# ImChouOWO/A-lightweight-Unsupervised-Feature-Extractor-

Hardware: NVIDIA B200
Metric: tracked frames/sec at N=64 boxes; ROIAlign achieved HBM GB/s vs B200 peak (higher is better)
Workload: dtype f32

## Files before the change

### a-lightweight-unsupervised-feature-extractor-_b200/csrc/tracker.cu

```cuda
#include <stdlib.h>
#include <string.h>

#include <new>

#include <cuda_fp16.h>

#include "assoc_cost.cuh"
#include "kalman.cuh"
#include "lsap.cuh"

namespace b200 {
namespace trk {

struct Span {
    int k;
    __device__ explicit Span(int kk) : k(kk) { B200_SPAN_BEGIN(k); }
    __device__ ~Span() { B200_SPAN_END(k); }
};

#ifdef B200_TRK_TIMING
__device__ long long g_timing[32];
#define TRK_STAMP(k) do { __syncthreads(); if (threadIdx.x == 0 && blockIdx.x == 0) g_timing[k] = clock64(); } while (0)
#define TRK_GSTAMP(k) do { __syncthreads(); if (threadIdx.x == 0 && blockIdx.x == 0 && blockIdx.y == 0) g_timing[16 + (k)] = (long long)::b200::gtime(); } while (0)
#else
// ... 68 lines not shown
    }
    return base;
}

__device__ __forceinline__ void load_kf(const Dev& d, size_t slot, double* x, double* P) {
    const double2* px = reinterpret_cast<const double2*>(d.kf_x + slot * 8);
    const double2* pP = reinterpret_cast<const double2*>(d.kf_P + slot * 64);
#pragma unroll
    for (int k = 0; k < 4; ++k) { const double2 v = px[k]; x[2 * k] = v.x; x[2 * k + 1] = v.y; }
#pragma unroll
    for (int k = 0; k < 32; ++k) { const double2 v = pP[k]; P[2 * k] = v.x; P[2 * k + 1] = v.y; }
}
__device__ __forceinline__ void store_kf(const Dev& d, size_t slot, const double* x, const double* P) {
    double2* px = reinterpret_cast<double2*>(d.kf_x + slot * 8);
    double2* pP = reinterpret_cast<double2*>(d.kf_P + slot * 64);
#pragma unroll
    for (int k = 0; k < 4; ++k) px[k] = make_double2(x[2 * k], x[2 * k + 1]);
#pragma unroll
    for (int k = 0; k < 32; ++k) pP[k] = make_double2(P[2 * k], P[2 * k + 1]);
}

__device__ inline void purge(const Dev& d, int s, int nl, int* scratch) {
    int* order = d.order + (size_t)s * d.MT;
    int* tmp = d.tmp + (size_t)s * d.MT;
    int* fl = d.free_list + (size_t)s * d.MT;
    int* hdr = d.hdr + s * kHdr;
    const size_t sb = (size_t)s * d.MT;
    for (int i = threadIdx.x; i < nl; i += blockDim.x) tmp[i] = order[i];
    __syncthreads();
    const int nfree = hdr[H_NFREE];
    const int keep = block_compact(nl, [&](int i) { return d.miss[sb + tmp[i]] <= d.max_age; },
                                   [&](int pos, int i) { order[pos] = tmp[i]; }, scratch);
    const int dead = block_compact(nl, [&](int i) { return d.miss[sb + tmp[i]] > d.max_age; },
                                   [&](int pos, int i) { fl[nfree + pos] = tmp[i]; }, scratch);
    if (threadIdx.x == 0) { hdr[H_NLIVE] = keep; hdr[H_NFREE] = nfree + dead; }
    __syncthreads();
}

__device__ inline void enqueue_cost_work(int2* work, int* counter, int s, int M, int N, int* scratch) {
    const int tiles = (N + cost::kTileN - 1) / cost::kTileN, total = M * tiles;
    if (total <= 0) return;
    __syncthreads();
    if (threadIdx.x == 0) scratch[0] = atomicAdd(counter, total);
    __syncthreads();
    const int base = scratch[0];
    for (int i = threadIdx.x; i < total; i += blockDim.x) work[base + i] = make_int2(s, (i / tiles) * 64 + i % tiles);
}

__device__ inline void prep_detections(const Dev& d, int s, int n, int part = 0, int nparts = 1) {
    const size_t db = (size_t)s * d.MD;
    const int tid = threadIdx.x;
    const int nw = blockDim.x >> 5, nt = blockDim.x;
    for (int j = part * nw + (tid >> 5); j < n; j += nparts * nw) {
        const float4 v = reinterpret_cast<const float4*>(d.embs + (db + j) * cost::kD)[tid & 31];
        reinterpret_cast<float4*>(d.det_unit + (db + j) * cost::kD)[tid & 31] = cost::unit_row(v);
    }
    for (int j = part * nt + tid; j < n; j += nparts * nt) {
        double b[4];
        float z[4];
#pragma unroll
        for (int k = 0; k < 4; ++k) { b[k] = d.boxes[(db + j) * 4 + k]; d.det_boxf[(db + j) * 4 + k] = (float)b[k]; }
        kf::box_to_z(b, z);
#pragma unroll
        for (int k = 0; k < 4; ++k) d.det_z[(db + j) * 4 + k] = z[k];
        d.det_conff[db + j] = (float)d.confs[db + j];
        d.det_used[db + j] = 0;
    }
}

__device__ inline void predict_slot(const Dev& d, size_t slot) {
    const float q[8] = {1.f, 1.f, 1.f, 1.f, 100.f, 100.f, 100.f, 100.f};
    const float rdiag[4] = {1.f, 1.f, 1.f, 1.f};
    double x[8], P[64], b[4];
    load_kf(d, slot, x, P);
    const int st = d.kf_stage[slot];
    kf::predict(x, P, st, q);
    store_kf(d, slot, x, P);
    kf::x_to_box(x, b);
#pragma unroll
    for (int k = 0; k < 4; ++k) { d.last_bbox[slot * 4 + k] = b[k]; d.prev_boxf[slot * 4 + k] = (float)b[k]; }
    d.prev_conff[slot] = (float)d.last_conf[slot];
    kf::Gate g;
    kf::gate_prepare(x, P, st, rdiag, &g);
#pragma unroll
    for (int k = 0; k < 16; ++k) d.gate_SI[slot * 16 + k] = g.SI[k];
}

__global__ void __launch_bounds__(kThreads) begin_kernel(Dev d) {
    Span span((d.frame_id[0] & 7) * 6 + 0);
    __shared__ int scratch[kThreads / 32];
    const int s = blockIdx.x, tid = threadIdx.x;
    int* hdr = d.hdr + s * kHdr;
    int* cnt = d.cnt + s * kHdr;
    int* res = d.result + (size_t)s * d.res_stride;
    const size_t sb = (size_t)s * d.MT, db = (size_t)s * d.MD;
    const int n = d.n_det[s], nl = hdr[H_NLIVE];
    int* order = d.order + sb;
    if (blockIdx.y == 1) {
        if (n <= 0) return;
        prep_detections(d, s, n);
        return;
    }
    if (s == 0 && tid == 0) d.wcount[2] = 0;
    if (n < 0) {
        if (tid == 0) {
            cnt[C_MODE] = MODE_SKIP;
            res[R_NMATCH] = res[R_NUT] = res[R_NUD] = res[R_STATUS] = res[R_M1] = res[R_M2] = 0;
            res[R_NLIVE] = nl;
            res[R_NEXT] = hdr[H_NEXT];
        }
        return;
    }
    if (n == 0) {
        int* ut = res_ut(d, res);
        for (int p = tid; p < nl; p += blockDim.x) {
            const size_t slot = sb + order[p];
            d.miss[slot] += 1;
            ut[p] = d.tid[slot];
        }
        __syncthreads();
        purge(d, s, nl, scratch);
        if (tid == 0) {
            cnt[C_MODE] = MODE_EMPTY;
            res[R_NMATCH] = 0; res[R_NUT] = nl; res[R_NUD] = 0; res[R_STATUS] = 0; res[R_M1] = res[R_M2] = 0;
            res[R_NLIVE] = hdr[H_NLIVE];
            res[R_NEXT] = hdr[H_NEXT];
        }
        return;
    }
    for (int p = tid; p < nl; p += blockDim.x) predict_slot(d, sb + order[p]);
    int* rm = d.rows_main + sb;
    int* rr = d.rows_reid + sb;
    const int M1 = block_compact(nl, [&](int i) { return d.miss[sb + order[i]] <= d.lost_reid_after; },
                                 [&](int pos, int i) { rm[pos] = order[i]; }, scratch);
    const int M2 = block_compact(nl, [&](int i) { return d.miss[sb + order[i]] > d.lost_reid_after; },
                                 [&](int pos, int i) { rr[pos] = order[i]; }, scratch);
    if (tid == 0) {
        cnt[C_M1] = M1; cnt[C_M2] = M2; cnt[C_NU] = 0; cnt[C_MODE] = MODE_NORMAL;
        cnt[C_NMATCH] = 0; cnt[C_NUT] = 0; cnt[C_STATUS] = 0;
    }
    enqueue_cost_work(d.work1, d.wcount + 0, s, M1, 1, scratch);
}

__device__ inline void cost2_item(const Dev& d, int s, int r, int j0, float* smem, int* s_idx) {
    const int tid = threadIdx.x, warp = tid >> 5, lane = tid & 31;
    const int N = d.cnt[s * kHdr + C_NU];
    const size_t sb = (size_t)s * d.MT, db = (size_t)s * d.MD;
    const size_t slot = sb + d.rows_reid[sb + r];
    int T = d.bank_len[slot];
    const float* rows = d.bank + slot * d.HIST * cost::kD;
    if (T <= 0) { rows = d.ema + slot * cost::kD; T = 1; }
    if (tid < cost::kTileN) {
        const int j = j0 + tid;
        s_idx[tid] = j < N ? d.ud1[db + j] : 0;
    }
    __syncthreads();
    const int tc = cost::bank_cap(T);
    float* sBank = smem;
    float* sDet = sBank + tc * cost::kD;
    float* sSim = sDet + cost::kTileN * cost::kDetStride;
    for (int t = warp; t < tc; t += cost::kThreads / 32) {
        float4 v = make_float4(0, 0, 0, 0);
        if (t < T) v = cost::unit_row(reinterpret_cast<const float4*>(rows + (size_t)t * cost::kD)[lane]);
        reinterpret_cast<float4*>(sBank + t * cost::kD)[lane] = v;
    }
    for (int j = warp; j < cost::kTileN; j += cost::kThreads / 32) {
// ... 82 lines not shown
        float pb[4];
#pragma unroll
        for (int k = 0; k < 4; ++k) pb[k] = d.prev_boxf[slot * 4 + k];
        const float pconf = d.prev_conff[slot];
        float inv0 = 0.0f, inv1 = 0.0f;
        bool have_norm = false;
        RowMin rmin;
        for (int j0 = 0; j0 < N; j0 += 32) {
            const int j = j0 + lane;
            bool alive = false;
            if (j < N) alive = !(kf::gate_d2(SI, xs, stage, d.det_z + (db + j) * 4) > d.maha_thr);
            unsigned todo = __ballot_sync(0xffffffffu, alive);
            float c_app = 0.0f;
            while (todo) {
                const int jl = __ffs(todo) - 1;
                todo &= todo - 1;
                const float4 dv = reinterpret_cast<const float4*>(d.det_unit + (db + j0 + jl) * cost::kD)[lane];
                float s0 = kNegInf, s1 = kNegInf;
                for (int t0 = 0; t0 < T; t0 += 8) {
                    float4 bv[8];
#pragma unroll
                    for (int u = 0; u < 8; ++u)
                        if (t0 + u < T) bv[u] = reinterpret_cast<const float4*>(rows + (size_t)(t0 + u) * cost::kD)[lane];
#pragma unroll
                    for (int u = 0; u < 8; ++u) {
                        const int t = t0 + u;
                        if (t >= T) break;
                        float p = bv[u].x * dv.x;
                        p = fmaf(bv[u].y, dv.y, p); p = fmaf(bv[u].z, dv.z, p); p = fmaf(bv[u].w, dv.w, p);
                        p = warp_sum(p);
                        if (!have_norm) {
                            float q = bv[u].x * bv[u].x;
                            q = fmaf(bv[u].y, bv[u].y, q); q = fmaf(bv[u].z, bv[u].z, q); q = fmaf(bv[u].w, bv[u].w, q);
                            q = warp_sum(q);
                            const float iv = __fdiv_rn(1.0f, __fadd_rn(sqrtf(q), 1e-12f));
                            if (lane == (t & 31)) { if (t < 32) inv0 = iv; else inv1 = iv; }
                        }
                        if (lane == (t & 31)) { if (t < 32) s0 = p; else s1 = p; }
                    }
                }
                have_norm = true;
                if (lane < T) s0 *= inv0;
                if (lane + 32 < T) s1 *= inv1;
                float sum = 0.0f;
                for (int q = 0; q < kk; ++q) {
                    const float mine = fmaxf(s0, s1);
                    const unsigned m = __reduce_max_sync(0xffffffffu, fkey(mine));
                    const unsigned who = __ballot_sync(0xffffffffu, fkey(mine) == m);
                    if (lane == __ffs(who) - 1) {
                        if (s0 >= s1) s0 = kNegInf; else s1 = kNegInf;
                    }
                    const unsigned bits = m ^ ((m >> 31) ? 0x80000000u : 0xffffffffu);
                    sum = __fadd_rn(sum, __uint_as_float(bits));
                }
                const float ca = __fsub_rn(1.0f, __fdiv_rn(sum, (float)kk));
                if (lane == jl) c_app = ca;
            }
            if (j < N) {
                float total_c = 1e9f;
                if (alive)
                    total_c = cost::pair_cost(pb, d.det_boxf + (db + j) * 4, pconf, d.det_conff[db + j], d.pw, c_app).total;
                d.C1[(sb + r) * d.MD + j] = total_c;
                d.C1T[(db + j) * d.MT + r] = total_c;
                rmin.see(total_c, j);
            }
        }
        rmin.finish(d.row_fc + sb + r, d.row_fv + sb + r, lane);
    }
}

__device__ __forceinline__ void transpose_reduce32(float (&p)[32]) {
    const int lane = threadIdx.x & 31;
#pragma unroll
    for (int o = 16; o > 0; o >>= 1) {
        const bool up = lane & o;
#pragma unroll
        for (int i = 0; i < o; ++i) {
            const float keep = up ? p[i + o] : p[i], send = up ? p[i] : p[i + o];
            p[i] = keep + __shfl_xor_sync(0xffffffffu, send, o);
        }
    }
}

template <bool FLY>
__device__ __forceinline__ void cost1_row32(const Dev& d, int s, int r, size_t slot, int N, int lane) {
    const float kNegInf = -__int_as_float(0x7f800000);
    const size_t sb = (size_t)s * d.MT, db = (size_t)s * d.MD;
    int T = d.bank_len[slot];
    const float* rows = d.bank + slot * d.HIST * cost::kD;
    if (T <= 0) { rows = d.ema + slot * cost::kD; T = 1; }
    const int kk = min(d.topk, T);
    double SI[16], xs[4];
#pragma unroll
    for (int k = 0; k < 16; ++k) SI[k] = d.gate_SI[slot * 16 + k];
#pragma unroll
    for (int k = 0; k < 4; ++k) xs[k] = d.kf_x[slot * 8 + k];
    const int stage = d.kf_stage[slot];
    float pb[4];
#pragma unroll
    for (int k = 0; k < 4; ++k) pb[k] = d.prev_boxf[slot * 4 + k];
    const float pconf = d.prev_conff[slot];
    float4 bv[32];
    float inv = 0.0f;
    bool have_bank = false;
    RowMin rmin;
    for (int j0 = 0; j0 < N; j0 += 32) {
        const int j = j0 + lane;
        bool alive = false;
        float zl[4], bf[4];
        float cf = 0.0f;
        if (j < N) {
            if (FLY) {
                double b[4];
#pragma unroll
                for (int k = 0; k < 4; ++k) { b[k] = d.boxes[(db + j) * 4 + k]; bf[k] = (float)b[k]; }
                kf::box_to_z(b, zl);
                cf = (float)d.confs[db + j];
                alive = !(kf::gate_d2(SI, xs, stage, zl) > d.maha_thr);
            } else {
                alive = !(kf::gate_d2(SI, xs, stage, d.det_z + (db + j) * 4) > d.maha_thr);
            }
        }
        unsigned todo = __ballot_sync(0xffffffffu, alive);
        float c_app = 0.0f;
        float4 dv_first = make_float4(0, 0, 0, 0);
        if (todo) {
            const int jf = __ffs(todo) - 1;
            if (FLY) dv_first = reinterpret_cast<const float4*>(d.embs + (db + j0 + jf) * cost::kD)[lane];
            else dv_first = reinterpret_cast<const float4*>(d.det_unit + (db + j0 + jf) * cost::kD)[lane];
        }
        if (todo && !have_bank) {
            float q[32];
#pragma unroll
            for (int t = 0; t < 32; ++t)
                bv[t] = t < T ? reinterpret_cast<const float4*>(rows + (size_t)t * cost::kD)[lane] : make_float4(0, 0, 0, 0);
#pragma unroll
            for (int t = 0; t < 32; ++t) {
                float a = bv[t].x * bv[t].x;
                a = fmaf(bv[t].y, bv[t].y, a); a = fmaf(bv[t].z, bv[t].z, a); a = fmaf(bv[t].w, bv[t].w, a);
                q[t] = a;
            }
            transpose_reduce32(q);
            inv = __fdiv_rn(1.0f, __fadd_rn(sqrtf(q[0]), 1e-12f));
            have_bank = true;
        }
        bool first = true;
        while (todo) {
            const int jl = __ffs(todo) - 1;
            todo &= todo - 1;
            float4 dv = dv_first;
            if (!first) {
                if (FLY) dv = reinterpret_cast<const float4*>(d.embs + (db + j0 + jl) * cost::kD)[lane];
                else dv = reinterpret_cast<const float4*>(d.det_unit + (db + j0 + jl) * cost::kD)[lane];
            }
            first = false;
            if (FLY) dv = cost::unit_row(dv);
            float p[32];
#pragma unroll
            for (int t = 0; t < 32; ++t) {
                float a = bv[t].x * dv.x;
                a = fmaf(bv[t].y, dv.y, a); a = fmaf(bv[t].z, dv.z, a); a = fmaf(bv[t].w, dv.w, a);
                p[t] = a;
            }
            transpose_reduce32(p);
            float sim = lane < T ? p[0] * inv : kNegInf;
            float sum = 0.0f;
            for (int q = 0; q < kk; ++q) {
                const unsigned m = __reduce_max_sync(0xffffffffu, fkey(sim));
                const unsigned who = __ballot_sync(0xffffffffu, fkey(sim) == m);
                if (lane == __ffs(who) - 1) sim = kNegInf;
                const unsigned bits = m ^ ((m >> 31) ? 0x80000000u : 0xffffffffu);
                sum = __fadd_rn(sum, __uint_as_float(bits));
            }
            const float ca = __fsub_rn(1.0f, __fdiv_rn(sum, (float)kk));
            if (lane == jl) c_app = ca;
        }
        if (j < N) {
            float total_c = 1e9f;
            if (alive) {
                if (FLY) total_c = cost::pair_cost(pb, bf, pconf, cf, d.pw, c_app).total;
                else total_c = cost::pair_cost(pb, d.det_boxf + (db + j) * 4, pconf, d.det_conff[db + j], d.pw, c_app).total;
            }
            d.C1[(sb + r) * d.MD + j] = total_c;
            d.C1T[(db + j) * d.MT + r] = total_c;
            rmin.see(total_c, j);
        }
    }
    rmin.finish(d.row_fc + sb + r, d.row_fv + sb + r, lane);
}

__global__ void __launch_bounds__(kCost1Warps * 32, 2) cost1_sparse32_kernel(Dev d) {
    Span span((d.frame_id[0] & 7) * 6 + 1);
    TRK_PDL_PROLOGUE();
    const int total = d.wcount[0];
    const int warp = threadIdx.x >> 5, lane = threadIdx.x & 31;
    for (int wi = blockIdx.x * kCost1Warps + warp; wi < total; wi += gridDim.x * kCost1Warps) {
        const int2 item = d.work1[wi];
        const int s = item.x, r = item.y >> 6;
        const size_t sb = (size_t)s * d.MT;
        cost1_row32<false>(d, s, r, sb + d.rows_main[sb + r], d.n_det[s], lane);
    }
}

__device__ inline void note_matches(const Dev& d, int s, int nm, const int* rows, const float* C, int ldc,
                                    const int* m_col, int reid_stage, int* scratch, int queue_base = -1) {
    if (nm <= 0) return;
    const size_t sb = (size_t)s * d.MT, db = (size_t)s * d.MD;
    const int frame = d.frame_id[s];
    int base = queue_base;
    if (queue_base < 0) {
        __syncthreads();
        if (threadIdx.x == 0) scratch[0] = atomicAdd(d.wcount + 2, nm);
        __syncthreads();
        base = scratch[0];
    }
    for (int qd = threadIdx.x; qd < nm; qd += blockDim.x) {
        const int r = d.m_row[sb + qd], j = d.m_det[sb + qd];
        const size_t slot = sb + rows[r];
        const float c = C[(size_t)r * ldc + m_col[qd]];
#pragma unroll
        for (int k = 0; k < 4; ++k) d.last_bbox[slot * 4 + k] = d.boxes[(db + j) * 4 + k];
        d.last_conf[slot] = d.confs[db + j];
        d.last_frame[slot] = frame;
        d.age[slot] += 1;
        d.miss[slot] = 0;
        d.last_cost[slot] = (double)c;
        d.upd_slot[base + qd] = (int)slot;
        d.upd_det[base + qd] = (int)(db + j);
        d.upd_cost[base + qd] = c;
        d.upd_flag[base + qd] = (uint8_t)reid_stage;
    }
}

constexpr int kUpdWarps = 4;

__device__ __forceinline__ void update_entries(const Dev& d, int first, int total, int wq, int nwq, double* scratch) {
    const int lane = threadIdx.x & 31, sub = lane & 7, grp = lane >> 3;
    double* sP = scratch + (size_t)grp * 96;
    double* sK = sP + 64;
    const float rdiag[4] = {1.f, 1.f, 1.f, 1.f};
    for (int w0 = wq * 4; w0 < total; w0 += nwq * 4) {
        const int idx = first + w0 + grp;
        const bool on = w0 + grp < total;
        size_t slot = 0, det = 0;
        int st = -1, reid = 0;
        double c = 0.0, conf = 0.0;
        if (on) {
            slot = (size_t)d.upd_slot[idx];
            det = (size_t)d.upd_det[idx];
            c = (double)d.upd_cost[idx];
            reid = d.upd_flag[idx];
            st = d.kf_stage[slot];
            conf = d.confs[det];
        }
        const float* z = d.det_z + det * 4;
        const double cmax = reid ? d.reid_only_cost_max : d.cost_update_max;
        int app = on && !(conf < d.conf_update_min) && !(c > cmax);
        const int nst = st < 2 ? st + 1 : 2;
        float4 e[4], o[4];
        size_t slots[4];
        int len[4], head[4];
#pragma unroll
        for (int u = 0; u < 4; ++u) {
            const bool on_u = __shfl_sync(0xffffffffu, (int)on, u * 8) != 0;
            const unsigned long long sl = __shfl_sync(0xffffffffu, (unsigned long long)slot, u * 8);
            const unsigned long long dt = __shfl_sync(0xffffffffu, (unsigned long long)det, u * 8);
            slots[u] = (size_t)sl;
            if (on_u) {
                e[u] = reinterpret_cast<const float4*>(d.det_unit + (size_t)dt * cost::kD)[lane];
                o[u] = reinterpret_cast<const float4*>(d.ema + slots[u] * cost::kD)[lane];
// ... 155 lines not shown
            n_match = block_compact(M, is_match, [&](int pos, int r) {
                const int jl = col[r], j = STAGE == 1 ? jl : d.ud1[db + jl];
                d.m_row[sb + pos] = r;
                d.m_det[sb + pos] = j;
                m_col[pos] = jl;
                d.det_used[db + j] = 1;
                out_m[2 * (match0 + pos)] = d.tid[sb + rows[r]];
                out_m[2 * (match0 + pos) + 1] = j;
            }, scratch);
            n_ut = block_compact(M, [&](int r) { return !is_match(r); }, [&](int pos, int r) {
                const size_t slot = sb + rows[r];
                d.miss[slot] += 1;
                out_ut[ut0 + pos] = d.tid[slot];
            }, scratch);
            __syncthreads();
            note_matches(d, s, n_match, rows, C, d.MD, m_col, STAGE == 2, scratch, OWNQ ? (int)sb + match0 : -1);
        }
    } else if (M > 0) {
        for (int r = tid; r < M; r += blockDim.x) {
            const size_t slot = sb + rows[r];
            d.miss[slot] += 1;
            out_ut[ut0 + r] = d.tid[slot];
        }
        n_ut = M;
        __syncthreads();
    }

    if (STAGE == 1) {
        if (failed) {
            if (tid == 0) { cnt[C_NU] = 0; cnt[C_NMATCH] = 0; cnt[C_NUT] = 0; }
            return true;
        }
        n_left = block_compact(N, [&](int j) { return d.det_used[db + j] == 0; },
                               [&](int pos, int j) { d.ud1[db + pos] = j; }, scratch);
        if (tid == 0) { cnt[C_NU] = n_left; cnt[C_NMATCH] = n_match; cnt[C_NUT] = n_ut; }
        if (!INLINE) enqueue_cost_work(d.work2, d.wcount + 1, s, n_left > 0 ? cnt[C_M2] : 0, n_left, scratch);
        TRK_STAMP(5);
        __syncthreads();
        return false;
    }

    if (failed) {
        if (tid == 0) {
            res[R_NMATCH] = match0; res[R_NUT] = ut0; res[R_NUD] = 0;
            res[R_NLIVE] = hdr[H_NLIVE]; res[R_NEXT] = hdr[H_NEXT]; res[R_STATUS] = cnt[C_STATUS];
            res[R_M1] = cnt[C_M1]; res[R_M2] = cnt[C_M2];
        }
        return true;
    }
    int* out_ud = res_ud(d, res);
    n_left = block_compact(N, [&](int jl) { return d.det_used[db + d.ud1[db + jl]] == 0; },
                           [&](int pos, int jl) { out_ud[pos] = d.ud1[db + jl]; }, scratch);
    int* born = d.born + db;
    const int want = block_compact(n_left, [&](int k) { return !(d.confs[db + out_ud[k]] < d.init_conf_min); },
                                   [&](int pos, int k) { born[pos] = out_ud[k]; }, scratch);
    const int nl = hdr[H_NLIVE];
    const int nb = spawn_tracks(d, s, born, want);
    purge(d, s, nl + nb, scratch);
    if (tid == 0) {
        res[R_NMATCH] = match0 + n_match;
        res[R_NUT] = ut0 + n_ut;
        res[R_NUD] = n_left;
        res[R_NLIVE] = hdr[H_NLIVE];
        res[R_NEXT] = hdr[H_NEXT];
        res[R_STATUS] = cnt[C_STATUS];
        res[R_M1] = cnt[C_M1];
        res[R_M2] = cnt[C_M2];
    }
    return true;
}

template <int STAGE>
__global__ void __launch_bounds__(kThreads) assign_kernel(Dev d, int smem_matrix_floats) {
    Span span((d.frame_id[0] & 7) * 6 + (STAGE == 1 ? 2 : 4));
    TRK_PDL_PROLOGUE();
    extern __shared__ __align__(16) unsigned char smem_raw[];
    assign_body<STAGE, false, false>(d, blockIdx.x, smem_raw, smem_matrix_floats);
}

#ifndef B200_TRK_FRONT_WARPS
#define B200_TRK_FRONT_WARPS 4
#endif
constexpr int kFrontWarps = B200_TRK_FRONT_WARPS;

__global__ void __launch_bounds__(kFrontWarps * 32, 2) front_kernel(Dev d) {
    Span span((d.frame_id[0] & 7) * 6 + 0);
    extern __shared__ __align__(16) int s_rows[];
    __shared__ int scratch[kThreads / 32];
    const int s = blockIdx.y, g = blockIdx.x, G = gridDim.x, tid = threadIdx.x, warp = tid >> 5, lane = tid & 31;
    TRK_GSTAMP(0);
    int* hdr = d.hdr + s * kHdr;
    int* cnt = d.cnt + s * kHdr;
    int* res = d.result + (size_t)s * d.res_stride;
    const size_t sb = (size_t)s * d.MT;
    const int n = d.n_det[s], nl = hdr[H_NLIVE];
    const int* order = d.order + sb;
    if (s == 0 && g == 0 && tid == 0) d.wcount[2] = 0;
    if (n < 0) {
        if (g == 0 && tid == 0) {
            cnt[C_MODE] = MODE_SKIP;
            res[R_NMATCH] = res[R_NUT] = res[R_NUD] = res[R_STATUS] = res[R_M1] = res[R_M2] = 0;
            res[R_NLIVE] = nl;
            res[R_NEXT] = hdr[H_NEXT];
        }
        return;
    }
    if (n == 0) {
        if (g != 0) return;
        int* ut = res_ut(d, res);
        for (int p = tid; p < nl; p += blockDim.x) {
            const size_t slot = sb + order[p];
            d.miss[slot] += 1;
            ut[p] = d.tid[slot];
        }
        __syncthreads();
        purge(d, s, nl, scratch);
        if (tid == 0) {
            cnt[C_MODE] = MODE_EMPTY;
            res[R_NMATCH] = 0; res[R_NUT] = nl; res[R_NUD] = 0; res[R_STATUS] = 0; res[R_M1] = res[R_M2] = 0;
            res[R_NLIVE] = hdr[H_NLIVE];
            res[R_NEXT] = hdr[H_NEXT];
        }
        return;
    }
    int* rm = s_rows;
    int* rr = s_rows + d.MT;
    const int M1 = block_compact(nl, [&](int i) { return d.miss[sb + order[i]] <= d.lost_reid_after; },
                                 [&](int pos, int i) { rm[pos] = order[i]; }, scratch);
    const int M2 = block_compact(nl, [&](int i) { return d.miss[sb + order[i]] > d.lost_reid_after; },
                                 [&](int pos, int i) { rr[pos] = order[i]; }, scratch);
    if (g == 0) {
        for (int i = tid; i < M1; i += blockDim.x) d.rows_main[sb + i] = rm[i];
        for (int i = tid; i < M2; i += blockDim.x) d.rows_reid[sb + i] = rr[i];
        if (tid == 0) {
            cnt[C_M1] = M1; cnt[C_M2] = M2; cnt[C_NU] = 0; cnt[C_MODE] = MODE_NORMAL;
            cnt[C_NMATCH] = 0; cnt[C_NUT] = 0; cnt[C_STATUS] = 0;
        }
    }
    TRK_GSTAMP(1);
    prep_detections(d, s, n, g, G);
    const int own1 = M1 > g ? (M1 - g + G - 1) / G : 0, own2 = M2 > g ? (M2 - g + G - 1) / G : 0;
    for (int i = tid; i < own1 + own2; i += blockDim.x)
        predict_slot(d, sb + (i < own1 ? rm[g + i * G] : rr[g + (i - own1) * G]));
    __syncthreads();
    TRK_GSTAMP(2);
    for (int i = warp; i < own1; i += kFrontWarps) {
        const int r = g + i * G;
        cost1_row32<true>(d, s, r, sb + rm[r], n, lane);
    }
    TRK_GSTAMP(3);
}

#ifndef B200_TRK_BACK_CLUSTER
#define B200_TRK_BACK_CLUSTER 4
#endif
constexpr int kBackCluster = B200_TRK_BACK_CLUSTER;

__device__ __forceinline__ unsigned cluster_ctarank() {
    unsigned r;
    asm volatile("mov.u32 %0, %%cluster_ctarank;" : "=r"(r));
    return r;
}
__device__ __forceinline__ unsigned cluster_nctarank() {
    unsigned r;
    asm volatile("mov.u32 %0, %%cluster_nctarank;" : "=r"(r));
    return r;
}
__device__ __forceinline__ void cluster_sync_all() {
    asm volatile("barrier.cluster.arrive.release.aligned;\n\tbarrier.cluster.wait.acquire.aligned;" ::: "memory");
}

template <bool UPDATES>
__global__ void __launch_bounds__(kThreads, UPDATES ? 1 : 2) back_kernel(Dev d, int smem_matrix_floats) {
    Span span((d.frame_id[0] & 7) * 6 + 2);
    TRK_PDL_PROLOGUE();
    extern __shared__ __align__(16) unsigned char smem_raw[];
    __shared__ int s_idx[cost::kTileN];
    const unsigned rank = cluster_ctarank(), nrank = cluster_nctarank();
    const int s = blockIdx.x / nrank, tid = threadIdx.x;
    const int* cnt = d.cnt + s * kHdr;
    TRK_GSTAMP(4);
    if (rank == 0) {
        if (!assign_body<1, true, UPDATES>(d, s, smem_raw, smem_matrix_floats)) {
            TRK_GSTAMP(5);
            const int M2 = cnt[C_M2], NU = cnt[C_NU];
            if (M2 > 0 && NU > 0) {
                const int tiles = (NU + cost::kTileN - 1) / cost::kTileN;
                for (int it = 0; it < M2 * tiles; ++it)
                    cost2_item(d, s, it / tiles, (it % tiles) * cost::kTileN, reinterpret_cast<float*>(smem_raw), s_idx);
            }
            __syncthreads();
        }
        TRK_GSTAMP(6);
        assign_body<2, true, UPDATES>(d, s, smem_raw, smem_matrix_floats);
        __syncthreads();
        TRK_GSTAMP(7);
    }
    if (!UPDATES) return;
    if (nrank > 1) cluster_sync_all();
    if (cnt[C_MODE] != MODE_NORMAL) return;
    const int total = d.result[(size_t)s * d.res_stride + R_NMATCH];
    const int warp = tid >> 5;
    update_entries(d, (int)((size_t)s * d.MT), total, (int)rank * (kThreads / 32) + warp, (int)nrank * (kThreads / 32),
                   reinterpret_cast<double*>(smem_raw) + (size_t)warp * 4 * 96);
    TRK_GSTAMP(8);
}


__device__ inline int find_slot(const Dev& d, int s, int nl, int track_id) {
    const size_t sb = (size_t)s * d.MT;
    int lo = 0, hi = nl - 1;
    while (lo <= hi) {
        const int mid = (lo + hi) >> 1, sl = d.order[sb + mid], t = d.tid[sb + sl];
        if (t == track_id) return sl;
        if (t < track_id) lo = mid + 1; else hi = mid - 1;
    }
    return -1;
}

__global__ void __launch_bounds__(kThreads) op_predict_kernel(Dev d, int s) {
    const size_t sb = (size_t)s * d.MT;
    const int nl = d.hdr[s * kHdr + H_NLIVE];
    for (int p = threadIdx.x; p < nl; p += blockDim.x) predict_slot(d, sb + d.order[sb + p]);
}

__global__ void __launch_bounds__(kThreads) op_mark_missed_kernel(Dev d, int s, const int* tids, int n) {
    const size_t sb = (size_t)s * d.MT;
    const int nl = d.hdr[s * kHdr + H_NLIVE];
    if (threadIdx.x == 0)
        for (int i = 0; i < n; ++i) {
            const int sl = find_slot(d, s, nl, tids[i]);
// ... 274 lines not shown
    PTR(row_fc, int); PTR(row_fv, float);
    PTR(rows_main, int); PTR(rows_reid, int); PTR(cnt, int); PTR(ud1, int); PTR(det_used, int); PTR(m_row, int);
    PTR(m_det, int); PTR(m_app, int); PTR(tmp, int); PTR(born, int); PTR(work1, int2); PTR(work2, int2); PTR(wcount, int);
    PTR(upd_slot, int); PTR(upd_det, int); PTR(upd_cost, float); PTR(upd_flag, uint8_t);
#undef PTR
    t->in_ndet = reinterpret_cast<int*>(base + o_in_ndet);
    t->in_frame = reinterpret_cast<int*>(base + o_in_frame);
    t->in_boxes = reinterpret_cast<double*>(base + o_in_boxes);
    t->in_confs = reinterpret_cast<double*>(base + o_in_confs);
    t->in_embs = reinterpret_cast<float*>(base + o_in_embs);
    t->dev_result = reinterpret_cast<int*>(base + o_result);
    t->pk_ndet = reinterpret_cast<int*>(base + o_pk_ndet);
    t->pk_boxes = reinterpret_cast<double*>(base + o_pk_boxes);
    t->pk_confs = reinterpret_cast<double*>(base + o_pk_confs);
    t->pk_embs = reinterpret_cast<float*>(base + o_pk_embs);
    t->pk_inv = reinterpret_cast<int*>(base + o_pk_inv);
    t->pk_over = reinterpret_cast<int*>(base + o_pk_over);
    t->in_bytes = in_end - o_in;
    t->res_bytes = S * (size_t)d.res_stride * sizeof(int);
    t->slot_bytes = ((t->in_bytes + 255) & ~(size_t)255) + ((t->res_bytes + 255) & ~(size_t)255);
    e = cudaMallocHost(&t->pinned, t->slot_bytes * b200_tracker::kRing);
    if (e == cudaSuccess) e = cudaMalloc(&t->ring_dev, t->slot_bytes * b200_tracker::kRing);
    if (e == cudaSuccess) e = cudaStreamCreateWithFlags(&t->up_stream, cudaStreamNonBlocking);
    if (e == cudaSuccess) e = cudaStreamCreateWithFlags(&t->down_stream, cudaStreamNonBlocking);
    for (int i = 0; e == cudaSuccess && i < b200_tracker::kRing; ++i) {
        e = cudaEventCreateWithFlags(&t->done[i], cudaEventDisableTiming);
        if (e == cudaSuccess) e = cudaEventCreateWithFlags(&t->up[i], cudaEventDisableTiming);
        if (e == cudaSuccess) e = cudaEventCreateWithFlags(&t->ran[i], cudaEventDisableTiming);
    }
    if (e != cudaSuccess) {
        b200_tracker_destroy(t);
        return fail(B200_ECUDA, "tracker_create: host ring / streams: %s", cudaGetErrorString(e));
    }
    d.pw = cost::PairWeights{(float)conf->w_app, (float)conf->w_bbox, (float)conf->w_conf, (float)conf->alpha,
                             (float)conf->beta, 1e-6f};
    d.maha_thr = conf->maha_thr; d.cost_max = conf->cost_max; d.conf_update_min = conf->conf_update_min;
    d.cost_update_max = conf->cost_update_max; d.reid_only_cost_max = conf->reid_only_cost_max;
    d.init_conf_min = conf->init_conf_min;
    d.ema_a = (float)conf->ema_alpha;
    d.ema_b = (float)(1.0 - conf->ema_alpha);
    d.topk = conf->emb_top_k; d.max_age = conf->max_age; d.lost_reid_after = conf->lost_reid_after;
    const int Rm = max_tracks < max_dets ? max_tracks : max_dets, Cm = max_tracks < max_dets ? max_dets : max_tracks;
    const size_t wb = lsap::work_bytes(Rm, Cm), budget = 200 * 1024;
    if (wb > budget) {
        b200_tracker_destroy(t);
        return fail(B200_EINVAL, "tracker_create: %d x %d exceeds the assignment kernel's shared memory", max_tracks, max_dets);
    }
    size_t mat = (size_t)Rm * Cm * sizeof(float);
    if (wb + mat > budget) mat = budget - wb;
    if (max_tracks <= 1024 && max_dets <= 256 && mat > 32 * 1024) mat = 32 * 1024;
    t->smem_matrix_floats = (int)(mat / sizeof(float));
    t->assign_smem = wb + mat;
    cudaFuncSetAttribute(trk::assign_kernel<1>, cudaFuncAttributeMaxDynamicSharedMemorySize, (int)budget);
    cudaFuncSetAttribute(trk::assign_kernel<2>, cudaFuncAttributeMaxDynamicSharedMemorySize, (int)budget);
    cudaFuncSetAttribute(trk::cost2_kernel, cudaFuncAttributeMaxDynamicSharedMemorySize, (int)cost::smem_bytes(cost::kMaxBank));
    trk::reset_kernel<<<n_streams, 128>>>(d);
    e = cudaDeviceSynchronize();
    if (e != cudaSuccess) {
        b200_tracker_destroy(t);
        return fail(B200_ECUDA, "tracker_create: %s", cudaGetErrorString(e));
    }
    g_launches.fetch_add(1);
    {
        int per_sm = 1, sms = kSMs, devid = 0;
        cudaGetDevice(&devid);
        cudaDeviceGetAttribute(&sms, cudaDevAttrMultiProcessorCount, devid);
        cudaOccupancyMaxActiveBlocksPerMultiprocessor(&per_sm, trk::cost2_kernel, cost::kThreads,
                                                      cost::smem_bytes(d.HIST));
        t->cost_grid = sms * (per_sm > 0 ? per_sm : 1);
        per_sm = 1;
        if (d.HIST <= 32)
            cudaOccupancyMaxActiveBlocksPerMultiprocessor(&per_sm, trk::cost1_sparse32_kernel, trk::kCost1Warps * 32, 0);
        else
            cudaOccupancyMaxActiveBlocksPerMultiprocessor(&per_sm, trk::cost1_sparse_kernel, trk::kCost1Warps * 32, 0);
        t->cost1_grid = sms * (per_sm > 0 ? per_sm : 1);
        t->upd_grid = sms * 2;
        const bool fits = max_tracks <= 512 && max_dets <= 256 && d.HIST <= 32;
        t->chain = !fits ? 6 : n_streams <= 8 ? 2 : 3;
        if (const char* e = getenv("B200TRACK_CHAIN")) {
            const int want = atoi(e);
            if (want == 6 || (fits && (want == 2 || want == 3))) t->chain = want;
        }
        if (t->chain != 6) {
            t->front_smem = sizeof(int) * 2 * (size_t)max_tracks;
            size_t bs = t->assign_smem;
            if (cost::smem_bytes(d.HIST) > bs) bs = cost::smem_bytes(d.HIST);
            if (sizeof(double) * (trk::kThreads / 32) * 4 * 96 > bs) bs = sizeof(double) * (trk::kThreads / 32) * 4 * 96;
            t->back_smem = bs;
            cudaFuncSetAttribute(trk::back_kernel<true>, cudaFuncAttributeMaxDynamicSharedMemorySize, (int)budget);
            cudaFuncSetAttribute(trk::back_kernel<false>, cudaFuncAttributeMaxDynamicSharedMemorySize, (int)budget);
            per_sm = 1;
            cudaOccupancyMaxActiveBlocksPerMultiprocessor(&per_sm, trk::front_kernel, trk::kFrontWarps * 32, t->front_smem);
            t->front_resident = sms * (per_sm > 0 ? per_sm : 1);
            if (const char* e = getenv("B200TRACK_FRONT_CTAS")) t->front_resident = atoi(e) > 0 ? atoi(e) : t->front_resident;
            if (const char* e = getenv("B200TRACK_UPD_CTAS")) t->upd_grid = atoi(e) > 0 ? atoi(e) : t->upd_grid;
        }
    }
    *out = t;
    return B200_OK;
}

extern "C" void b200_tracker_destroy(b200_tracker* t) {
    if (!t) return;
    if (t->up_stream) { cudaStreamSynchronize(t->up_stream); cudaStreamDestroy(t->up_stream); }
    if (t->down_stream) { cudaStreamSynchronize(t->down_stream); cudaStreamDestroy(t->down_stream); }
    for (int i = 0; i < b200_tracker::kRing; ++i) {
        if (t->done[i]) cudaEventDestroy(t->done[i]);
        if (t->up[i]) cudaEventDestroy(t->up[i]);
        if (t->ran[i]) cudaEventDestroy(t->ran[i]);
    }
    cudaFreeHost(t->pinned);
    cudaFree(t->ring_dev);
    cudaFree(t->arena);
    delete t;
}

extern "C" int b200_tracker_reset(b200_tracker* t, void* stream) {
    B200_REQUIRE(t, "tracker_reset: null handle");
    trk::reset_kernel<<<t->d.S, 128, 0, as_stream(stream)>>>(t->d);
    return check_launch("reset_kernel");
}

extern "C" int b200_tracker_result_stride(const b200_tracker* t) { return t ? t->d.res_stride : 0; }

extern "C" int b200_tracker_live_counts(b200_tracker* t, int32_t* n_live_host, int32_t* next_id_host, void* stream) {
    B200_REQUIRE(t, "tracker_live_counts: null handle");
    cudaStream_t st = as_stream(stream);
    const int S = t->d.S;
    int* h = static_cast<int*>(malloc(sizeof(int) * trk::kHdr * (size_t)S));
    B200_REQUIRE(h, "tracker_live_counts: out of host memory");
    cudaError_t e = cudaMemcpyAsync(h, t->d.hdr, sizeof(int) * trk::kHdr * (size_t)S, cudaMemcpyDeviceToHost, st);
    if (e == cudaSuccess) e = cudaStreamSynchronize(st);
    if (e != cudaSuccess) {
        free(h);
        return fail(B200_ECUDA, "tracker_live_counts: %s", cudaGetErrorString(e));
    }
    for (int s = 0; s < S; ++s) {
        if (n_live_host) n_live_host[s] = h[s * trk::kHdr + trk::H_NLIVE];
        if (next_id_host) next_id_host[s] = h[s * trk::kHdr + trk::H_NEXT];
    }
    free(h);
    return B200_OK;
}

extern "C" int b200_tracker_step(b200_tracker* t, const int32_t* n_det, const double* boxes, const double* confs,
                                 const float* embs, const int32_t* frame_id, int32_t* result, void* stream) {
    B200_REQUIRE(t && n_det && boxes && confs && embs && frame_id && result, "tracker_step: null pointer");
    cudaStream_t st = as_stream(stream);
    trk::Dev d = t->d;
    d.n_det = n_det; d.boxes = boxes; d.confs = confs; d.embs = embs; d.frame_id = frame_id; d.result = result;
    const size_t csm = cost::smem_bytes(d.HIST);
    const int cost_grid = t->cost_grid;
    int rc;
    if (t->chain != 6) {
        int G = t->front_resident / d.S;
        const int gmax = (d.MT + 3) / 4;
        G = G < 1 ? 1 : G > gmax ? gmax : G;
        trk::front_kernel<<<dim3(G, d.S), trk::kFrontWarps * 32, t->front_smem, st>>>(d);
        if ((rc = check_launch("trk front_kernel"))) return rc;
        if (t->chain == 3) {
            trk::back_kernel<false><<<d.S, trk::kThreads, t->assign_smem > cost::smem_bytes(d.HIST) ? t->assign_smem
                                                                                                    : cost::smem_bytes(d.HIST), st>>>(
                d, t->smem_matrix_floats);
            if ((rc = check_launch("trk back_kernel<false>"))) return rc;
            trk::update_kernel<<<t->upd_grid, trk::kUpdWarps * 32, 0, st>>>(d);
            return check_launch("trk update_kernel");
        }
// ... 417 lines not shown
```

Before: 265,900.

## Prefetch track feature banks via bulk async copies and split Kalman predict across lanes

The front kernel now issues cp.async.bulk loads of each warp's next track feature bank into a shared-memory ring, gated by mbarriers, so the bank fetch overlaps with detection prep and the predict step instead of sitting on each row's critical path. The cost row reads bank vectors from shared memory rather than holding 32 float4 registers. Kalman predict is also split so 8 lanes each handle one state row, exchanging rows via shuffles, rather than one thread per slot. This adds shared memory use that can lower occupancy, plus an alignment check at creation time.

New measurement: 267,600 (median of 6 runs). About the same (+0.6%).

```diff
diff --git a/a-lightweight-unsupervised-feature-extractor-_b200/csrc/tracker.cu b/a-lightweight-unsupervised-feature-extractor-_b200/csrc/tracker.cu
--- a/a-lightweight-unsupervised-feature-extractor-_b200/csrc/tracker.cu
+++ b/a-lightweight-unsupervised-feature-extractor-_b200/csrc/tracker.cu
@@ -174,6 +174,66 @@
     d.prev_conff[slot] = (float)d.last_conf[slot];
     kf::Gate g;
     kf::gate_prepare(x, P, st, rdiag, &g);
+#pragma unroll
+    for (int k = 0; k < 16; ++k) d.gate_SI[slot * 16 + k] = g.SI[k];
+}
+
+template <typename TX, typename TP>
+__device__ __forceinline__ void predict_row_t(double& x, double (&P)[8], double xu, const double (&Pu)[8], int i) {
+    if (i < 4) {
+        x = (double)((TX)x + (TX)xu);
+#pragma unroll
+        for (int j = 0; j < 8; ++j) P[j] = (double)((TP)P[j] + (TP)Pu[j]);
+    }
+#pragma unroll
+    for (int j = 0; j < 4; ++j) P[j] = (double)((TP)P[j] + (TP)P[j + 4]);
+    const float q = i < 4 ? 1.f : 100.f;
+#pragma unroll
+    for (int j = 0; j < 8; ++j)
+        if (j == i) P[j] = (double)((TP)P[j] + (TP)q);
+}
+
+__device__ __forceinline__ void predict_slot8(const Dev& d, size_t slot, bool on) {
+    const int lane = threadIdx.x & 31, i = lane & 7, base = lane & ~7;
+    double x = 0.0, P[8];
+    int st = 0;
+#pragma unroll
+    for (int j = 0; j < 8; ++j) P[j] = 0.0;
+    if (on) {
+        x = d.kf_x[slot * 8 + i];
+        const double2* pP = reinterpret_cast<const double2*>(d.kf_P + slot * 64 + i * 8);
+#pragma unroll
+        for (int k = 0; k < 4; ++k) { const double2 v = pP[k]; P[2 * k] = v.x; P[2 * k + 1] = v.y; }
+        st = d.kf_stage[slot];
+    }
+    double Pu[8];
+    const double xu = __shfl_down_sync(0xffffffffu, x, 4, 8);
+#pragma unroll
+    for (int j = 0; j < 8; ++j) Pu[j] = __shfl_down_sync(0xffffffffu, P[j], 4, 8);
+    if (st == 0) predict_row_t<float, float>(x, P, xu, Pu, i);
+    else if (st == 1) predict_row_t<float, double>(x, P, xu, Pu, i);
+    else predict_row_t<double, double>(x, P, xu, Pu, i);
+    double xg[4], Pg[32];
+#pragma unroll
+    for (int k = 0; k < 4; ++k) xg[k] = __shfl_sync(0xffffffffu, x, base + k);
+#pragma unroll
+    for (int r = 0; r < 4; ++r)
+#pragma unroll
+        for (int j = 0; j < 4; ++j) Pg[r * 8 + j] = __shfl_sync(0xffffffffu, P[j], base + r);
+    if (!on) return;
+    d.kf_x[slot * 8 + i] = x;
+    double2* pP = reinterpret_cast<double2*>(d.kf_P + slot * 64 + i * 8);
+#pragma unroll
+    for (int k = 0; k < 4; ++k) pP[k] = make_double2(P[2 * k], P[2 * k + 1]);
+    if (i != 0) return;
+    const float rdiag[4] = {1.f, 1.f, 1.f, 1.f};
+    double b[4];
+    kf::x_to_box(xg, b);
+#pragma unroll
+    for (int k = 0; k < 4; ++k) { d.last_bbox[slot * 4 + k] = b[k]; d.prev_boxf[slot * 4 + k] = (float)b[k]; }
+    d.prev_conff[slot] = (float)d.last_conf[slot];
+    kf::Gate g;
+    kf::gate_prepare(xg, Pg, st, rdiag, &g);
 #pragma unroll
     for (int k = 0; k < 16; ++k) d.gate_SI[slot * 16 + k] = g.SI[k];
 }
@@ -422,8 +482,28 @@
     }
 }
 
+__device__ __forceinline__ unsigned smem_addr(const void* p) { return (unsigned)__cvta_generic_to_shared(p); }
+__device__ __forceinline__ void mbar_init(unsigned bar, unsigned count) {
+    asm volatile("mbarrier.init.shared::cta.b64 [%0], %1;\n" ::"r"(bar), "r"(count) : "memory");
+}
+__device__ __forceinline__ void mbar_wait(unsigned bar, unsigned parity) {
+    asm volatile(
+        "{\n\t.reg .pred p;\n\t"
+        "WAIT_%=:\n\t"
+        "mbarrier.try_wait.parity.shared::cta.b64 p, [%0], %1;\n\t"
+        "@p bra DONE_%=;\n\t"
+        "bra WAIT_%=;\n\t"
+        "DONE_%=:\n\t}\n" ::"r"(bar), "r"(parity) : "memory");
+}
+__device__ __forceinline__ void bulk_load(unsigned dst, const void* src, unsigned bytes, unsigned bar) {
+    asm volatile("mbarrier.arrive.expect_tx.shared::cta.b64 _, [%0], %1;\n" ::"r"(bar), "r"(bytes) : "memory");
+    asm volatile("cp.async.bulk.shared::cluster.global.mbarrier::complete_tx::bytes [%0], [%1], %2, [%3];\n"
+                 ::"r"(dst), "l"(src), "r"(bytes), "r"(bar) : "memory");
+}
+
 template <bool FLY>
-__device__ __forceinline__ void cost1_row32(const Dev& d, int s, int r, size_t slot, int N, int lane) {
+__device__ __forceinline__ void cost1_row32(const Dev& d, int s, int r, size_t slot, int N, int lane,
+                                            const float4* sbank = nullptr, unsigned bar = 0, unsigned parity = 0) {
     const float kNegInf = -__int_as_float(0x7f800000);
     const size_t sb = (size_t)s * d.MT, db = (size_t)s * d.MD;
     int T = d.bank_len[slot];
@@ -471,13 +551,18 @@
         }
         if (todo && !have_bank) {
             float q[32];
-#pragma unroll
-            for (int t = 0; t < 32; ++t)
-                bv[t] = t < T ? reinterpret_cast<const float4*>(rows + (size_t)t * cost::kD)[lane] : make_float4(0, 0, 0, 0);
+            if constexpr (FLY) {
+                mbar_wait(bar, parity);
+            } else {
+#pragma unroll
+                for (int t = 0; t < 32; ++t)
+                    bv[t] = t < T ? reinterpret_cast<const float4*>(rows + (size_t)t * cost::kD)[lane] : make_float4(0, 0, 0, 0);
+            }
 #pragma unroll
             for (int t = 0; t < 32; ++t) {
-                float a = bv[t].x * bv[t].x;
-                a = fmaf(bv[t].y, bv[t].y, a); a = fmaf(bv[t].z, bv[t].z, a); a = fmaf(bv[t].w, bv[t].w, a);
+                const float4 b = t >= T ? make_float4(0, 0, 0, 0) : FLY ? sbank[t * 32 + lane] : bv[t];
+                float a = b.x * b.x;
+                a = fmaf(b.y, b.y, a); a = fmaf(b.z, b.z, a); a = fmaf(b.w, b.w, a);
                 q[t] = a;
             }
             transpose_reduce32(q);
@@ -498,8 +583,9 @@
             float p[32];
 #pragma unroll
             for (int t = 0; t < 32; ++t) {
-                float a = bv[t].x * dv.x;
-                a = fmaf(bv[t].y, dv.y, a); a = fmaf(bv[t].z, dv.z, a); a = fmaf(bv[t].w, dv.w, a);
+                const float4 b = t >= T ? make_float4(0, 0, 0, 0) : FLY ? sbank[t * 32 + lane] : bv[t];
+                float a = b.x * dv.x;
+                a = fmaf(b.y, dv.y, a); a = fmaf(b.z, dv.z, a); a = fmaf(b.w, dv.w, a);
                 p[t] = a;
             }
             transpose_reduce32(p);
@@ -526,6 +612,7 @@
             rmin.see(total_c, j);
         }
     }
+    if (FLY && !have_bank) mbar_wait(bar, parity);
     rmin.finish(d.row_fc + sb + r, d.row_fv + sb + r, lane);
 }
 
@@ -847,10 +934,30 @@
 #define B200_TRK_FRONT_WARPS 4
 #endif
 constexpr int kFrontWarps = B200_TRK_FRONT_WARPS;
+#ifndef B200_TRK_FRONT_SLOTS
+#define B200_TRK_FRONT_SLOTS 1
+#endif
+constexpr int kFrontSlotsPerWarp = B200_TRK_FRONT_SLOTS;
+constexpr int kFrontSlots = kFrontWarps * kFrontSlotsPerWarp;
+
+__host__ __device__ inline size_t front_ring_offset(int MT) { return ((size_t)2 * MT * sizeof(int) + 127) & ~(size_t)127; }
+__host__ __device__ inline size_t front_bars_offset(int MT, int HIST) {
+    return front_ring_offset(MT) + (size_t)kFrontSlots * HIST * cost::kD * sizeof(float);
+}
+__host__ __device__ inline size_t front_smem_bytes(int MT, int HIST) {
+    return front_bars_offset(MT, HIST) + kFrontSlots * sizeof(unsigned long long);
+}
+
+__device__ __forceinline__ void fetch_bank(const Dev& d, size_t slot, unsigned dst, unsigned bar) {
+    int T = d.bank_len[slot];
+    const float* src = d.bank + slot * d.HIST * cost::kD;
+    if (T <= 0) { src = d.ema + slot * cost::kD; T = 1; }
+    bulk_load(dst, src, (unsigned)T * cost::kD * sizeof(float), bar);
+}
 
 __global__ void __launch_bounds__(kFrontWarps * 32, 2) front_kernel(Dev d) {
     Span span((d.frame_id[0] & 7) * 6 + 0);
-    extern __shared__ __align__(16) int s_rows[];
+    extern __shared__ __align__(128) int s_rows[];
     __shared__ int scratch[kThreads / 32];
     const int s = blockIdx.y, g = blockIdx.x, G = gridDim.x, tid = threadIdx.x, warp = tid >> 5, lane = tid & 31;
     TRK_GSTAMP(0);
@@ -902,16 +1009,40 @@
             cnt[C_NMATCH] = 0; cnt[C_NUT] = 0; cnt[C_STATUS] = 0;
         }
     }
+    const int own1 = M1 > g ? (M1 - g + G - 1) / G : 0, own2 = M2 > g ? (M2 - g + G - 1) / G : 0;
+    const int nmine = own1 > warp ? (own1 - warp + kFrontWarps - 1) / kFrontWarps : 0;
+    float* ring = reinterpret_cast<float*>(reinterpret_cast<char*>(s_rows) + front_ring_offset(d.MT)) +
+                  (size_t)warp * kFrontSlotsPerWarp * d.HIST * cost::kD;
+    const unsigned bars = smem_addr(reinterpret_cast<char*>(s_rows) + front_bars_offset(d.MT, d.HIST)) +
+                          warp * kFrontSlotsPerWarp * 8u;
+    const auto row_slot = [&](int m) { return sb + rm[g + (warp + m * kFrontWarps) * G]; };
+    if (lane == 0) {
+#pragma unroll
+        for (int k = 0; k < kFrontSlotsPerWarp; ++k) mbar_init(bars + 8u * k, 1);
+        asm volatile("fence.mbarrier_init.release.cluster;\n" ::: "memory");
+        for (int m = 0; m < kFrontSlotsPerWarp && m < nmine; ++m)
+            fetch_bank(d, row_slot(m), smem_addr(ring + (size_t)m * d.HIST * cost::kD), bars + 8u * m);
+    }
+    __syncwarp();
     TRK_GSTAMP(1);
     prep_detections(d, s, n, g, G);
-    const int own1 = M1 > g ? (M1 - g + G - 1) / G : 0, own2 = M2 > g ? (M2 - g + G - 1) / G : 0;
-    for (int i = tid; i < own1 + own2; i += blockDim.x)
-        predict_slot(d, sb + (i < own1 ? rm[g + i * G] : rr[g + (i - own1) * G]));
+    for (int i0 = 0; i0 < own1 + own2; i0 += blockDim.x / 8) {
+        const int i = i0 + (tid >> 3);
+        const bool on = i < own1 + own2;
+        predict_slot8(d, on ? sb + (i < own1 ? rm[g + i * G] : rr[g + (i - own1) * G]) : 0, on);
+    }
     __syncthreads();
     TRK_GSTAMP(2);
-    for (int i = warp; i < own1; i += kFrontWarps) {
-        const int r = g + i * G;
-        cost1_row32<true>(d, s, r, sb + rm[r], n, lane);
+    for (int m = 0; m < nmine; ++m) {
+        const int r = g + (warp + m * kFrontWarps) * G, k = m % kFrontSlotsPerWarp;
+        float* buf = ring + (size_t)k * d.HIST * cost::kD;
+        cost1_row32<true>(d, s, r, sb + rm[r], n, lane, reinterpret_cast<const float4*>(buf), bars + 8u * k,
+                          (unsigned)(m / kFrontSlotsPerWarp) & 1u);
+        __syncwarp();
+        if (lane == 0 && m + kFrontSlotsPerWarp < nmine) {
+            asm volatile("fence.proxy.async.shared::cta;\n" ::: "memory");
+            fetch_bank(d, row_slot(m + kFrontSlotsPerWarp), smem_addr(buf), bars + 8u * k);
+        }
     }
     TRK_GSTAMP(3);
 }
@@ -1352,7 +1483,12 @@
             if (want == 6 || (fits && (want == 2 || want == 3))) t->chain = want;
         }
         if (t->chain != 6) {
-            t->front_smem = sizeof(int) * 2 * (size_t)max_tracks;
+            if ((reinterpret_cast<uintptr_t>(d.bank) | reinterpret_cast<uintptr_t>(d.ema)) & 15) {
+                b200_tracker_destroy(t);
+                return fail(B200_ECUDA, "tracker_create: bank / EMA arrays are not 16-byte aligned");
+            }
+            t->front_smem = trk::front_smem_bytes(max_tracks, d.HIST);
+            cudaFuncSetAttribute(trk::front_kernel, cudaFuncAttributeMaxDynamicSharedMemorySize, (int)budget);
             size_t bs = t->assign_smem;
             if (cost::smem_bytes(d.HIST) > bs) bs = cost::smem_bytes(d.HIST);
             if (sizeof(double) * (trk::kThreads / 32) * 4 * 96 > bs) bs = sizeof(double) * (trk::kThreads / 32) * 4 * 96;
```
